# fircarpediem/LSS2_Multimodal_nu

Hardware: AMD Instinct MI355X
Metric: BEV frames/sec (6-cam 352x128 -> 200x200x64), full hot path: CamEncode lift + splat + BevEncode (higher is better)
Workload: dtype bf16; 1 GPU; BASELINE configs[1]: model_BEV_TXT LSS hot path, batch=4/GPU, 6 cams 352x128, D=41, 200x200x64 BEV -> BevEncode -> 200x200x4, trunk (EfficientNet) not included: features are the input; batch_per_gpu=4, global_batch=4, parallelism=dp1 (sample-sharded, no collective), precision=bf16

## Files before the change

include/lss_hip.h:

```cpp
#ifndef LSS_HIP_H_
#define LSS_HIP_H_

#include <stddef.h>
#include <stdint.h>

#ifdef __cplusplus
extern "C" {
#endif

#define LSS_ABI_VERSION 1

#define LSS_E_NULL (-1)
#define LSS_E_SHAPE (-2)
#define LSS_E_LAYOUT (-3)
#define LSS_E_ALIGN (-4)
#define LSS_E_WORKSPACE (-5)
#define LSS_E_RCCL_BASE (-100)

#define LSS_BEV_NCHW_F32 0
#define LSS_BEV_NHWC_F32 1
#define LSS_BEV_NHWC_BF16 2

#define LSS_DT_F32 0
#define LSS_DT_BF16 1
// ... 45 lines not shown
int lss_lift_splat_fwd(const float* feat, const int32_t* vox_list, const int32_t* entries,
                       int B, int N, int D, int fH, int fW, int C, int X, int Y, int Z,
                       void* bev, int layout, void* stream);

int lss_lift_splat_bwd(const void* grad_bev, int layout, const int32_t* voxel,
                       const float* depth, const float* feat, int B, int N, int D,
                       int fH, int fW, int C, int X, int Y, int Z, float* g_logits,
                       void* stream);

int lss_segmented_sum(const float* x, const int32_t* seg_start, int M, int C, float* y,
                      void* stream);

int lss_add_pos_fwd(const void* x, const float* pos, int B, int T, int C, int dt, void* q,
                    void* stream);

#define LSS_VALUE_NHWC 0
#define LSS_VALUE_HEAD_MAJOR 1
int lss_deform_attn_fwd(const void* value, int value_layout, const float* offsets_logits,
                        const float* token_bias, const float* ref_x, const float* ref_y, int B, int H,
                        int W, int n_heads, int n_points, int C, int dt, void* out, void* stream);

int lss_deform_attn_pts_fwd(const float* value, const float* offsets_logits, const float* ref_pts,
                            long long ref_bstride, int B, int H, int W, int n_heads, int n_points, int C,
                            float* out, void* stream);

int lss_deform_attn_bwd(const float* value, const float* offsets_logits, const float* ref_pts,
                        long long ref_bstride, const float* d_out, int B, int H, int W, int n_heads,
                        int n_points, int C, void* workspace, size_t workspace_bytes, float* d_value,
                        float* d_offsets_logits, void* stream);
size_t lss_deform_attn_bwd_workspace_bytes(int B, int H, int W);

int lss_layernorm_fwd(const void* x, int x_dt, const float* gamma, const float* beta,
                      long long rows, int C, float eps, void* y, int y_dt, void* stream);

size_t lss_conv2d_packed_weight_bytes(int Cout, int Cin, int KH, int KW, int dt);
int lss_conv2d_pack_weights(const float* w_oihw, int Cout, int Cin, int KH, int KW,
                            int dt, void* w_packed, void* stream);
int lss_conv2d_fwd(const void* x, const void* x2, const void* w_packed,
                   const float* scale, const float* shift, const void* residual,
                   void* y, float* stats, int B, int H, int W, int Cx, int C2, int up,
                   int Cout, int KH, int KW, int stride, int pad, int relu, int dt,
                   void* stream);

int lss_conv2d_ring_ok(int B, int H, int W, int Cx, int C2, int up, int Cout, int head_n);
size_t lss_conv2d_ring_packed_weight_bytes(int Cout, int Cin);
int lss_conv2d_pack_weights_ring(const float* w_oihw, int Cout, int Cin, void* w_packed, void* stream);
int lss_conv2d_pack_weights_ring_dgrad(const float* w_oihw, int Cout, int Cin, void* w_packed, void* stream);
int lss_conv2d_ring_timeouts(void);

int lss_conv2d_ks_ok(int B, int H, int W, int Cin, int Cout);
size_t lss_conv2d_ks_packed_weight_bytes(int Cout, int Cin);
int lss_conv2d_pack_weights_ks(const float* w_oihw, int Cout, int Cin, void* w_packed, void* stream);
int lss_conv2d_pack_weights_ks_dgrad(const float* w_oihw, int Cout, int Cin, void* w_packed, void* stream);

int lss_conv2d_pack_weights_dgrad(const float* w_oihw, int Cout, int Cin, int KH, int KW, int dt,
                                  void* w_packed, void* stream);
size_t lss_conv2d_wgrad_workspace_bytes(int B, int H, int W, int Cin, int Cout);
int lss_conv2d_wgrad(const void* x, const void* dy, int B, int H, int W, int Cin, int Cout,
                     void* workspace, size_t workspace_bytes, float* dw_oihw, void* stream);
int lss_conv2d_wgrad_timeouts(void);
int lss_conv2d_s2_dgrad_taps(int K, int pad);
int lss_conv2d_pack_weights_s2_dgrad(const float* w_oihw, int Cout, int Cin, int K, int pad, void* w_packed, void* stream);
size_t lss_conv2d_wgrad4x4_workspace_bytes(int B, int H, int W, int Cin, int Cout);
int lss_conv2d_wgrad4x4(const void* xs, const void* dy, int B, int H, int W, int Cin, int Cout,
                        void* workspace, size_t workspace_bytes, float* dw16, void* stream);

int lss_upsample_cat_nhwc(const void* x, const void* x2, int B, int H, int W, int Cx, int C2, int up,
                          void* out, void* stream);
int lss_upsample_bwd_nhwc(const void* g, int B, int H, int W, int Cx, int Ct, int c_off, int up,
                          void* dx, void* stream);

size_t lss_bn_train_workspace_bytes(long long M, int C);
int lss_bn_train_fwd(const void* z, const void* residual, long long M, int C, const float* gamma,
                     const float* beta, float* running_mean, float* running_var, float momentum,
                     float eps, int relu, void* workspace, void* y, float* save_mean,
                     float* save_invstd, void* stream);
int lss_bn_train_bwd(const void* dy, const void* y, const void* z, long long M, int C,
                     const float* gamma, const float* save_mean, const float* save_invstd, int relu,
                     void* workspace, void* dz, void* dres, float* dgamma, float* dbeta, void* stream);

int lss_bn_partial_sums(const void* z, const void* dy, const void* y, const float* mean, const float* invstd,
                        long long M, int C, int relu, int mode, void* workspace, float* sums, void* stream);
int lss_bn_train_fwd_from_sums(const void* z, const void* residual, long long M, int C, const float* sums,
                               long long M_total, const float* gamma, const float* beta, float* running_mean,
                               float* running_var, float momentum, float eps, int relu, void* workspace,
                               void* y, float* save_mean, float* save_invstd, void* stream);
int lss_bn_train_bwd_from_sums(const void* dy, const void* y, const void* z, long long M, int C,
                               const float* sums, long long M_total, const float* gamma,
                               const float* save_mean, const float* save_invstd, int relu, void* workspace,
                               void* dz, void* dres, float* dgamma, float* dbeta, void* stream);

int lss_conv_bn_act_train_fwd(const void* x1, const void* x2, const float* w_oihw, const float* gamma,
                              const float* beta, const void* residual, float* running_mean,
                              float* running_var, void* w_packed, void* z, void* y, float* save_mean,
                              float* save_invstd, void* bn_workspace, int B, int H, int W, int Cx, int C2,
                              int up, int Cout, float momentum, float eps, int relu, void* stream);
int lss_conv_bn_act_train_pack(const float* w_oihw, int B, int H, int W, int Cx, int C2, int up, int Cout, int dgrad,
                               void* w_packed, void* stream);
int lss_conv_bn_act_train_bwd(const void* dy, const void* y, const void* z, const void* x1, const void* x2,
                              const float* w_oihw, const float* gamma, const float* save_mean,
                              const float* save_invstd, void* bn_workspace, void* wgrad_workspace,
                              size_t wgrad_workspace_bytes, void* w_dgrad, void* dz, void* dres,
                              float* dgamma, float* dbeta, void* gcat, void* g1, void* xcat, float* dw,
                              int B, int H, int W, int Cx, int C2, int up, int Cout, int relu,
                              void* stream);

// ... 118 lines not shown
```

lss2_multimodal_nu_amd/_native.py:

```python
import ctypes
import os

import torch

_HERE = os.path.dirname(os.path.abspath(__file__))
LIB_PATH = os.environ.get("LSS_HIP_LIB") or os.path.join(_HERE, "csrc", "liblss_hip.so")

BEV_NCHW_F32, BEV_NHWC_F32, BEV_NHWC_BF16 = 0, 1, 2
DT_F32, DT_BF16 = 0, 1
ACT_NONE, ACT_RELU, ACT_GELU, OUT_F32, OUT_HEAD_MAJOR32, W_RING, W_KS = 0, 1, 2, 16, 32, 64, 128
VALUE_NHWC, VALUE_HEAD_MAJOR = 0, 1

_vp, _i, _sz = ctypes.c_void_p, ctypes.c_int, ctypes.c_size_t

SIGNATURES = {
    "lss_abi_version": (_i, []),
    "lss_error_string": (ctypes.c_char_p, [_i]),
    "lss_points_to_voxels": (_i, [_vp] * 7 + [_i] * 8 + [_vp, _vp, _vp, _vp]),
    "lss_geom_to_voxels": (_i, [_vp, _vp, _vp] + [_i] * 5 + [_vp, _vp, _vp]),
    "lss_bucket_points": (_i, [_vp, _vp, _i, _i, _i, _i, _vp, _vp, _vp, _vp, _vp]),
    "lss_depthnet_softmax_fwd": (_i, [_vp, _vp, _vp, _i, _i, _i, _i, _i, _vp, _vp, _i, _vp]),
    "lss_camencode_v2_fwd": (_i, [_vp, _i, _vp, _vp, _i, _vp, _vp, _vp] + [_i] * 7 + [_vp, _vp, _vp]),
    "lss_depth_fuse_softmax_fwd": (_i, [_vp] * 5 + [_i] * 6 + [_vp, _vp]),
    "lss_add_pos_fwd": (_i, [_vp, _vp, _i, _i, _i, _i, _vp, _vp]),
    "lss_deform_attn_fwd": (_i, [_vp, _i] + [_vp] * 4 + [_i] * 7 + [_vp, _vp]),
    "lss_deform_attn_pts_fwd": (_i, [_vp] * 3 + [ctypes.c_longlong] + [_i] * 6 + [_vp, _vp]),
    "lss_deform_attn_bwd": (_i, [_vp] * 3 + [ctypes.c_longlong, _vp] + [_i] * 6 + [_vp, _sz, _vp, _vp, _vp]),
    "lss_deform_attn_bwd_workspace_bytes": (_sz, [_i] * 3),
    "lss_layernorm_fwd": (_i, [_vp, _i, _vp, _vp, ctypes.c_longlong, _i, ctypes.c_float, _vp, _i, _vp]),
    "lss_depthnet_voxels_fwd": (_i, [_vp] * 10 + [_i] * 10 + [_vp] * 5),
    "lss_linear_res_ln_fwd": (_i, [_vp] * 4 + [ctypes.c_longlong, _i, _vp, _vp, _vp, ctypes.c_float, _vp, _vp]),
    "lss_ffn_fused_fwd": (_i, [_vp] * 5 + [ctypes.c_longlong, _i, _i, _vp, _vp, _vp, ctypes.c_float, _vp, _vp]),
    "lss_depthnet_voxels_hostcal_fwd": (_i, [_vp] * 7 + [_i] * 10 + [_vp] * 5),
    "lss_lift_splat_forward_hostcal": (_i, [_vp] * 7 + [_i] * 10 + [_vp] * 8 + [_i, _vp]),
    "lss_lift_splat_fwd": (_i, [_vp] * 3 + [_i] * 9 + [_vp, _i, _vp]),
    "lss_lift_splat_bwd": (_i, [_vp, _i, _vp, _vp, _vp] + [_i] * 9 + [_vp, _vp]),
    "lss_segmented_sum": (_i, [_vp, _vp, _i, _i, _vp, _vp]),
    "lss_conv2d_packed_weight_bytes": (_sz, [_i] * 5),
    "lss_conv2d_pack_weights": (_i, [_vp, _i, _i, _i, _i, _i, _vp, _vp]),
    "lss_conv2d_fwd": (_i, [_vp] * 8 + [_i] * 13 + [_vp]),
    "lss_conv2d_ring_ok": (_i, [_i] * 8),
    "lss_conv2d_ring_packed_weight_bytes": (_sz, [_i, _i]),
    "lss_conv2d_pack_weights_ring": (_i, [_vp, _i, _i, _vp, _vp]),
    "lss_conv2d_pack_weights_ring_dgrad": (_i, [_vp, _i, _i, _vp, _vp]),
    "lss_conv2d_ks_ok": (_i, [_i] * 5),
    "lss_conv2d_ks_packed_weight_bytes": (_sz, [_i, _i]),
    "lss_conv2d_pack_weights_ks": (_i, [_vp, _i, _i, _vp, _vp]),
    "lss_conv2d_pack_weights_ks_dgrad": (_i, [_vp, _i, _i, _vp, _vp]),
    "lss_gather_pack": (_i, [_vp, _i, _vp]),
    "lss_conv_bn_act_train_pack": (_i, [_vp] + [_i] * 8 + [_vp, _vp]),
    "lss_clip_adam_partials": (ctypes.c_longlong, [_vp, _i]),
    "lss_clip_adam_step": (_i, [_vp, _i, _vp, _vp, ctypes.c_longlong] + [ctypes.c_float] * 6 + [_vp]),
    "lss_conv2d_wgrad_timeouts": (_i, []),
    "lss_conv2d_ring_timeouts": (_i, []),
    "lss_conv2d_pack_weights_dgrad": (_i, [_vp, _i, _i, _i, _i, _i, _vp, _vp]),
    "lss_conv2d_wgrad_workspace_bytes": (_sz, [_i] * 5),
    "lss_conv2d_wgrad": (_i, [_vp, _vp, _i, _i, _i, _i, _i, _vp, _sz, _vp, _vp]),
    "lss_conv2d_wgrad4x4_workspace_bytes": (_sz, [_i] * 5),
    "lss_conv2d_s2_dgrad_taps": (_i, [_i, _i]),
    "lss_conv2d_pack_weights_s2_dgrad": (_i, [_vp, _i, _i, _i, _i, _vp, _vp]),
    "lss_conv2d_wgrad4x4": (_i, [_vp, _vp, _i, _i, _i, _i, _i, _vp, _sz, _vp, _vp]),
    "lss_upsample_cat_nhwc": (_i, [_vp, _vp, _i, _i, _i, _i, _i, _i, _vp, _vp]),
    "lss_upsample_bwd_nhwc": (_i, [_vp, _i, _i, _i, _i, _i, _i, _i, _vp, _vp]),
    "lss_bn_train_workspace_bytes": (_sz, [ctypes.c_longlong, _i]),
    "lss_bn_train_fwd": (_i, [_vp, _vp, ctypes.c_longlong, _i, _vp, _vp, _vp, _vp, ctypes.c_float, ctypes.c_float, _i,
                              _vp, _vp, _vp, _vp, _vp]),
    "lss_bn_train_bwd": (_i, [_vp, _vp, _vp, ctypes.c_longlong, _i, _vp, _vp, _vp, _i, _vp, _vp, _vp, _vp, _vp, _vp]),
    "lss_bn_partial_sums": (_i, [_vp] * 5 + [ctypes.c_longlong, _i, _i, _i, _vp, _vp, _vp]),
    "lss_bn_train_fwd_from_sums": (_i, [_vp, _vp, ctypes.c_longlong, _i, _vp, ctypes.c_longlong, _vp, _vp, _vp, _vp,
                                        ctypes.c_float, ctypes.c_float, _i, _vp, _vp, _vp, _vp, _vp]),
    "lss_bn_train_bwd_from_sums": (_i, [_vp, _vp, _vp, ctypes.c_longlong, _i, _vp, ctypes.c_longlong, _vp, _vp, _vp, _i,
                                        _vp, _vp, _vp, _vp, _vp, _vp]),
    "lss_conv_bn_act_train_fwd": (_i, [_vp] * 14 + [_i] * 7 + [ctypes.c_float, ctypes.c_float, _i, _vp]),
    "lss_conv_bn_act_train_bwd": (_i, [_vp] * 11 + [_sz] + [_vp] * 9 + [_i] * 8 + [_vp]),
    "lss_weighted_ce_fwd": (_i, [_vp, _vp, _vp, _i, _i, ctypes.c_longlong, _vp, _vp, _vp, _vp]),
    "lss_weighted_ce_bwd": (_i, [_vp, _vp, _vp, _i, _i, ctypes.c_longlong, _vp, _vp, _vp, _vp]),
    "lss_conv2d_s2d_packed_weight_bytes": (_sz, [_i] * 4),
    "lss_conv2d_pack_weights_s2d": (_i, [_vp, _i, _i, _i, _i, _vp, _vp]),
    "lss_conv2d_s2_fwd": (_i, [_vp] * 7 + [_i] * 8 + [_vp]),
    "lss_conv2d_head_fwd": (_i, [_vp] * 8 + [_i] * 9 + [_vp]),
    "lss_conv2d_s2_dual_fwd": (_i, [_vp] * 6 + [_i] * 9 + [_vp]),
    "lss_conv2d_sequence": (_i, [_vp, _i, _vp]),
    "lss_lift_splat_forward": (_i, [_vp] * 10 + [_i] * 10 + [_vp] * 8 + [_i, _i, _vp]),
    "lss_region_pipeline_ok": (_i, [_i] * 9),
    "lss_lift_splat_from_heads": (_i, [_vp] * 9 + [_i] * 9 + [_vp] * 6 + [_i, _vp]),
    "lss_lift_splat_direct_bytes": (_sz, [_i] * 9),
    "lss_lift_splat_forward_desc": (_i, [_vp, _vp]),
    "lss_head_ce_workspace_bytes": (_sz, [_i]),
    "lss_head_ce_fwd": (_i, [_vp] * 5 + [ctypes.c_longlong, _i, _i, _vp, _vp, _vp, _vp]),
    "lss_head_ce_bwd": (_i, [_vp] * 5 + [ctypes.c_longlong, _i, _i] + [_vp] * 7),
    "lss_head1x1_fwd": (_i, [_vp] * 3 + [ctypes.c_longlong, ctypes.c_longlong, _i, _i, _vp, _vp]),
    "lss_head1x1_bwd": (_i, [_vp] * 4 + [ctypes.c_longlong, ctypes.c_longlong, _i, _i] + [_vp] * 5),
    "lss_rccl_unique_id_bytes": (_sz, []),
    "lss_rccl_version": (_i, [_vp]),
    "lss_rccl_get_unique_id": (_i, [_vp]),
    "lss_rccl_comm_init": (_i, [_vp, _i, _i, _vp]),
    "lss_allreduce_bucket": (_i, [_vp, _vp, ctypes.c_longlong, _vp]),
    "lss_rccl_comm_destroy": (_i, [_vp]),
    "lss_nchw_f32_to_nhwc": (_i, [_vp, _vp, _i, _i, _i, _i, _i, _vp]),
    "lss_nhwc_to_nchw_f32": (_i, [_vp, _vp, _i, _i, _i, _i, _i, _vp]),
}
# ... 81 lines not shown
```

lss2_multimodal_nu_amd/csrc/conv_ks.hip:

```cpp
#include <stdlib.h>

#include "lss_common.h"

namespace {

constexpr int KS_ROWS = 7;
constexpr int KS_POSB = 64;
constexpr int KS_LDS_MAX = 160 * 1024;

__device__ __attribute__((aligned(128))) unsigned char lss_ks_zero_page[128];

__device__ __forceinline__ void ks_glds16(const void* gsrc, void* lds_wave_base) {
  __builtin_amdgcn_global_load_lds((const __attribute__((address_space(1))) void*)gsrc,
                                   (__attribute__((address_space(3))) void*)lds_wave_base, 16, 0, 0);
}

struct KsArgs {
  const unsigned short* x;
  const unsigned char* w;
  const float* scale;
  const float* shift;
  const unsigned short* residual;
  unsigned short* y;
  int B, H, W, Cin, Cout, relu, wt;
// ... 217 lines not shown
    const int cb = r / nks;
    const int m = l & 15, kq = l >> 4;
    const int co = cb * 32 + 8 * (m >> 2) + 4 * ct + (m & 3);
    const int ci = (S / 9) * 32 + kq * 8 + j;
    out[e] = lss_f2bf(dgrad ? w[((size_t)ci * Cout + co) * 9 + (8 - S % 9)] : w[((size_t)co * Cin + ci) * 9 + (S % 9)]);
  }
}

struct KsPlan {
  int ok, PB, npb, nposp, ncb, lds, grid, variant;
};

KsPlan ks_plan(int B, int H, int W, int Cin, int Cout) {
  KsPlan p = {};
  if (B <= 0 || H <= 0 || W < 4 || Cout <= 0 || Cout % 32 != 0) return p;
  if (Cin == 256) { p.variant = 0; p.PB = 80; }
  else if (Cin == 128) { p.variant = 1; p.PB = 160; }
  else if (Cin == 64) { p.variant = 2; p.PB = 320; }
  else return p;
  const long long HW = (long long)H * W;
  if (p.PB > 4 * W + 1) return p;
  p.npb = (int)((HW + p.PB - 1) / p.PB);
  p.ncb = Cout / 32;
  p.nposp = (KS_ROWS * (W + 2) + 31) / 32 * 32;
  const int patch = (Cin / 32) * p.nposp * KS_POSB;
  if (patch > 112 * 1024) return p;
  const int ntile = p.PB / 16;
  const int red = (p.variant == 2 ? 2 : 4) * ntile * 2 * 1024;
  p.lds = patch > red ? patch : red;
  if (p.lds > KS_LDS_MAX) return p;
  const long long grid = (long long)B * p.npb * p.ncb;
  if (grid < 64 || grid > 512) return p;
  if ((long long)B * HW * (Cin > Cout ? Cin : Cout) >= (1LL << 30)) return p;
  p.grid = (int)grid;
  p.ok = 1;
  return p;
}

template <int KSW, int NKW, int PXT>
int ks_launch(const KsPlan& p, const KsArgs& a, hipStream_t st) {
  static bool attr_set[64] = {};
  int dev = -1;
  if (hipGetDevice(&dev) != hipSuccess || dev < 0 || dev >= 64) dev = -1;
  if (dev < 0 || !attr_set[dev]) {
    hipError_t e = hipFuncSetAttribute(reinterpret_cast<const void*>(conv_ks_kernel<KSW, NKW, PXT>),
                                       hipFuncAttributeMaxDynamicSharedMemorySize, KS_LDS_MAX);
    if (e != hipSuccess) return (int)e;
    if (dev >= 0) attr_set[dev] = true;
  }
  hipLaunchKernelGGL((conv_ks_kernel<KSW, NKW, PXT>), dim3(p.grid), dim3(256), p.lds, st, a);
  return lss_launch_status();
}

}

extern "C" int lss_conv2d_ks_ok(int B, int H, int W, int Cin, int Cout) {
  if (const char* e = getenv("LSS_CONV_KS"))
    if (atoi(e) == 0) return 0;
  return ks_plan(B, H, W, Cin, Cout).ok;
}

extern "C" size_t lss_conv2d_ks_packed_weight_bytes(int Cout, int Cin) {
  if (Cout <= 0 || Cout % 32 != 0 || (Cin != 64 && Cin != 128 && Cin != 256)) return 0;
  return (size_t)Cout * Cin * 9 * 2;
}

extern "C" int lss_conv2d_pack_weights_ks(const float* w_oihw, int Cout, int Cin, void* w_packed, void* stream) {
  LSS_CHECK_PTR(w_oihw); LSS_CHECK_PTR(w_packed);
  if (lss_conv2d_ks_packed_weight_bytes(Cout, Cin) == 0) return LSS_E_SHAPE;
  const size_t n = (size_t)Cout * Cin * 9;
  const int grid = (int)((n + 255) / 256 > 4096 ? 4096 : (n + 255) / 256);
  hipLaunchKernelGGL(pack_weights_ks_kernel, dim3(grid), dim3(256), 0, lss_stream(stream), w_oihw, Cout, Cin,
                     reinterpret_cast<unsigned short*>(w_packed), 0);
  return lss_launch_status();
}

extern "C" int lss_conv2d_pack_weights_ks_dgrad(const float* w_oihw, int Cout, int Cin, void* w_packed, void* stream) {
  LSS_CHECK_PTR(w_oihw); LSS_CHECK_PTR(w_packed);
  if (lss_conv2d_ks_packed_weight_bytes(Cin, Cout) == 0) return LSS_E_SHAPE;
  const size_t n = (size_t)Cout * Cin * 9;
  const int grid = (int)((n + 255) / 256 > 4096 ? 4096 : (n + 255) / 256);
  hipLaunchKernelGGL(pack_weights_ks_kernel, dim3(grid), dim3(256), 0, lss_stream(stream), w_oihw, Cin, Cout,
                     reinterpret_cast<unsigned short*>(w_packed), 1);
  return lss_launch_status();
}

int lss_conv_ks_launch(const void* x, const void* w_ks, const float* scale, const float* shift, const void* residual,
                       void* y, int B, int H, int W, int Cin, int Cout, int relu, int wt, hipStream_t st) {
  const KsPlan p = ks_plan(B, H, W, Cin, Cout);
  if (!p.ok) return LSS_E_SHAPE;
  if (relu != 0 && relu != 1) return LSS_E_LAYOUT;
  if (((reinterpret_cast<uintptr_t>(x) | reinterpret_cast<uintptr_t>(y) | reinterpret_cast<uintptr_t>(w_ks) |
        reinterpret_cast<uintptr_t>(residual)) & 15) != 0)
    return LSS_E_ALIGN;
  KsArgs a;
  a.x = reinterpret_cast<const unsigned short*>(x);
  a.w = reinterpret_cast<const unsigned char*>(w_ks);
  a.scale = scale; a.shift = shift;
  a.residual = reinterpret_cast<const unsigned short*>(residual);
  a.y = reinterpret_cast<unsigned short*>(y);
  a.B = B; a.H = H; a.W = W; a.Cin = Cin; a.Cout = Cout; a.relu = relu; a.wt = wt;
  a.PB = p.PB; a.npb = p.npb; a.nposp = p.nposp; a.ncb = p.ncb;
  {
    const char* e = getenv("LSS_KS_STAMPS");
    a.stamps = e ? reinterpret_cast<unsigned long long*>(strtoull(e, nullptr, 16)) : nullptr;
  }
  if (p.variant == 0) return ks_launch<18, 4, 5>(p, a, st);
  if (p.variant == 1) return ks_launch<9, 4, 10>(p, a, st);
  return ks_launch<9, 2, 10>(p, a, st);
}
```

lss2_multimodal_nu_amd/csrc/conv_mfma.hip:

```cpp
#include <stdlib.h>

#include "lss_common.h"

int lss_linear_bf16_launch(const void* x, const void* w, const float* scale, const float* shift,
                           const void* residual, void* y, long long M, int N, int K, int act,
                           int out_f32, int group_hw, hipStream_t st);

int lss_conv_ring_launch(const void* x, const void* x2, const void* w_ring, const float* scale, const float* shift,
                         void* y, const float* head_w, const float* head_b, float* head_out, int head_n, int B, int H,
                         int W, int Cx, int C2, int up, int Cout, int relu, int wt, hipStream_t st);

int lss_conv_ks_launch(const void* x, const void* w_ks, const float* scale, const float* shift, const void* residual,
                       void* y, int B, int H, int W, int Cin, int Cout, int relu, int wt, hipStream_t st);

namespace {

struct ConvArgs {
  const void* x;
  const void* x2;
  const void* w;
  const float* scale;
  const float* shift;
  const void* residual;
  void* y;
// ... 1161 lines not shown
  a.y = nullptr; a.stats = nullptr;
  a.B = B; a.H = H; a.W = W; a.Cx = Cx; a.C2 = C2; a.up = up;
  a.Hin = H * up; a.Win = W * up; a.Cin = Cx + C2;
  a.Cout = Cout; a.KH = 3; a.KW = 3; a.stride = 1; a.pad = 1;
  a.Ho = a.Hin; a.Wo = a.Win;
  const long long M = (long long)B * a.Ho * a.Wo;
  if (M >= (1LL << 31)) return LSS_E_SHAPE;
  a.M = (int)M;
  a.relu = relu & 3;
  a.out_f32 = 0;
  a.wt = (getenv("LSS_CONV_WT") == nullptr || atoi(getenv("LSS_CONV_WT")) != 0) &&
         (unsigned long long)a.M * a.Cout * 2 < (1ULL << 31);
  a.y2 = nullptr; a.split = 0; a.relu_n = a.Cout;
  a.head_w = head_w; a.head_b = head_b; a.head_out = out; a.head_n = head_n;
  a.ry = a.Hin > 1 ? (float)(H - 1) / (float)(a.Hin - 1) : 0.f;
  a.rx = a.Win > 1 ? (float)(W - 1) / (float)(a.Win - 1) : 0.f;
  const bool fused = (up > 1) || (C2 > 0);
  const int tilesX = lss_cdiv(a.Wo, 16), tilesY = lss_cdiv(a.Ho, Cout == 64 ? 16 : 8);
  dim3 g(tilesX * tilesY * B, 1);
  hipStream_t st = lss_stream(stream);
  bool kc32 = fused && a.Cx % 32 == 0 && a.C2 % 32 == 0;
  if (const char* e = getenv("LSS_CONV_KC")) kc32 = kc32 && atoi(e) == 32;
  if (fused && kc32) {
    a.src_lds = conv_src_lds_ok(a);
    hipLaunchKernelGGL((conv_lds_kernel<2, 128, 1, 3, 3, 1, 32, 1, true>), g, dim3(256), 0, st, a, tilesX, tilesY);
  }
  else if (fused)
    hipLaunchKernelGGL((conv_lds_kernel<2, 128, 1, 3, 3, 1, 64, 1, true>), g, dim3(256), 0, st, a, tilesX, tilesY);
  else if (Cout == 64)
    hipLaunchKernelGGL((conv_lds_kernel<2, 64, 0, 3, 3, 1, 64, 1, true>), g, dim3(256), 0, st, a, tilesX, tilesY);
  else
    hipLaunchKernelGGL((conv_lds_kernel<2, 128, 0, 3, 3, 1, 64, 1, true>), g, dim3(256), 0, st, a, tilesX, tilesY);
  return lss_launch_status();
}

extern "C" int lss_conv2d_sequence(const lss_conv_launch_t* L, int n, void* stream) {
  LSS_CHECK_PTR(L);
  if (n < 0) return LSS_E_SHAPE;
  for (int i = 0; i < n; ++i) {
    const lss_conv_launch_t& c = L[i];
    int rc;
    if (c.kind == 0)
      rc = lss_conv2d_fwd(c.x, c.x2, c.w, c.scale, c.shift, c.residual, c.y, c.stats, c.B, c.H, c.W, c.Cx,
                          c.C2, c.up, c.Cout, c.KH, c.KW, c.stride, c.pad, c.relu, c.dt, stream);
    else if (c.kind == 1)
      rc = lss_conv2d_s2_fwd(c.x, c.w, c.scale, c.shift, c.residual, c.y, c.stats, c.B, c.H, c.W, c.Cx,
                             c.Cout, c.KH, c.pad, c.relu, stream);
    else if (c.kind == 2)
      rc = lss_conv2d_head_fwd(c.x, c.x2, c.w, c.scale, c.shift, c.head_w, c.head_b, c.head_out, c.B, c.H,
                               c.W, c.Cx, c.C2, c.up, c.Cout, c.head_n, c.relu, stream);
    else if (c.kind == 3)
      rc = lss_conv2d_s2_dual_fwd(c.x, c.w, c.scale, c.shift, c.y, c.y2, c.B, c.H, c.W, c.Cx, c.Cout, c.split, c.KH,
                                  c.pad, c.relu, stream);
    else
      rc = LSS_E_LAYOUT;
    if (rc != 0) return rc;
  }
  return 0;
}
```

lss2_multimodal_nu_amd/modules.py:

```python
import os

import torch
from torch import nn
from torch.nn import functional as F

from . import ops

_PRECISIONS = {"bf16": ops.DT_BF16, "fp32": ops.DT_F32}


def default_precision():
    p = os.environ.get("LSS_PRECISION", "bf16")
    if p not in _PRECISIONS:
        raise ValueError("LSS_PRECISION must be one of %s" % sorted(_PRECISIONS))
    return p


_warned_eval_autograd = set()


def _needs_autograd(module, *inputs):
    if not torch.is_grad_enabled():
        return False
    in_grad = any(t is not None and torch.is_tensor(t) and t.requires_grad for t in inputs)
# ... 628 lines not shown
    def forward(self, x):
        return self.get_eff_depth(x)

    def _load_from_state_dict(self, state_dict, prefix, local_metadata, strict, missing_keys, unexpected_keys,
                              error_msgs):
        if getattr(self, "trunk", None) is None:
            drop = [k for k in state_dict if k.startswith(prefix + "trunk.")]
            if drop:
                import warnings
                warnings.warn("%d '%strunk.*' checkpoint entries ignored: this Encoder was built without a trunk"
                              % (len(drop), prefix), stacklevel=3)
                for k in drop:
                    del state_dict[k]
        super()._load_from_state_dict(state_dict, prefix, local_metadata, strict, missing_keys, unexpected_keys,
                                      error_msgs)


class BasicBlock(nn.Module):

    def __init__(self, inplanes, planes, stride=1):
        super().__init__()
        self.conv1 = nn.Conv2d(inplanes, planes, 3, stride, 1, bias=False)
        self.bn1 = nn.BatchNorm2d(planes)
        self.relu = nn.ReLU(inplace=True)
        self.conv2 = nn.Conv2d(planes, planes, 3, 1, 1, bias=False)
        self.bn2 = nn.BatchNorm2d(planes)
        self.downsample = None
        if stride != 1 or inplanes != planes:
            self.downsample = nn.Sequential(nn.Conv2d(inplanes, planes, 1, stride, bias=False),
                                            nn.BatchNorm2d(planes))
        self._f1 = _FoldedConv(self.conv1, self.bn1)
        self._f2 = _FoldedConv(self.conv2, self.bn2)
        self._fd = _FoldedConv(self.downsample[0], self.downsample[1]) if self.downsample is not None else None

    def forward(self, x):
        idt = x if self.downsample is None else _train_bn_act(self.downsample[1], _train_conv(self.downsample[0], x), relu=False)
        out = _train_conv_bn_act(self.conv1, self.bn1, x, relu=True)
        return _train_conv_bn_act(self.conv2, self.bn2, out, relu=True, residual=idt)

    def _dual(self, dt):
        key = self._f1._key(dt) + self._fd._key(dt)
        if getattr(self, "_dual_key", None) != key:
            with torch.no_grad():
                w1, s1, b1 = self._f1.get(dt)
                _, sd, bd = self._fd.get(dt)
                wd = self.downsample[0].weight.detach().float()
                frame = wd.new_zeros(wd.shape[0], wd.shape[1], 3, 3)
                frame[:, :, 1, 1] = wd[:, :, 0, 0]
                self._dual_pack = (torch.cat([w1, ops.pack_conv_weight_s2d(frame.contiguous(), 1)], 1).contiguous(),
                                   torch.cat([s1, sd]).contiguous(), torch.cat([b1, bd]).contiguous())
            self._dual_key = key
        return self._dual_pack

    def _nhwc(self, x, dt):
        c1 = self.conv1
        if (self._fd is not None and dt == ops.DT_BF16 and c1.stride == (2, 2) and self._f1._s2d(dt)
                and self.downsample[0].stride == (2, 2) and c1.out_channels % 128 == 0
                and os.environ.get("LSS_NO_DUAL") is None):
            w, scale, shift = self._dual(dt)
            t, idt = ops.conv2d_s2_dual_nhwc(x, w, scale, shift, c1.out_channels, relu=True)
            return self._f2.run(t, dt, relu=True, residual=idt)
        idt = x if self._fd is None else self._fd.run(x, dt, relu=False)
        t = self._f1.run(x, dt, relu=True)
        return self._f2.run(t, dt, relu=True, residual=idt)


def _resnet18_layer(inplanes, planes, stride):
    return nn.Sequential(BasicBlock(inplanes, planes, stride), BasicBlock(planes, planes, 1))


class BevEncode(nn.Module):

    def __init__(self, inC, outC, precision=None):
        super().__init__()
        self.conv1 = nn.Conv2d(inC, 64, kernel_size=7, stride=2, padding=3, bias=False)
        self.bn1 = nn.BatchNorm2d(64)
        self.relu = nn.ReLU(inplace=True)
        self.layer1 = _resnet18_layer(64, 64, 1)
        self.layer2 = _resnet18_layer(64, 128, 2)
        self.layer3 = _resnet18_layer(128, 256, 2)
        for m in self.modules():
            if isinstance(m, nn.Conv2d):
                nn.init.kaiming_normal_(m.weight, mode="fan_out", nonlinearity="relu")
            elif isinstance(m, nn.BatchNorm2d):
                nn.init.constant_(m.weight, 1)
                nn.init.constant_(m.bias, 0)
        for m in self.modules():
            if isinstance(m, BasicBlock):
                nn.init.constant_(m.bn2.weight, 0)
        self.conv1.reset_parameters()
        self.up1 = Up(64 + 256, 256, scale_factor=4, precision=precision)
        self.up2 = nn.Sequential(
            nn.Upsample(scale_factor=2, mode="bilinear", align_corners=True),
            nn.Conv2d(256, 128, kernel_size=3, padding=1, bias=False),
            nn.BatchNorm2d(128),
            nn.ReLU(inplace=True),
            nn.Conv2d(128, outC, kernel_size=1, padding=0),
        )
        self.precision = precision
        self._plans = {}
        self._stem = _FoldedConv(self.conv1, self.bn1)
        self._up2a = _FoldedConv(self.up2[1], self.up2[2])
        self._up2b = _FoldedConv(self.up2[4], None)

    def features(self, x):
        if _native_training() and x.is_cuda:
            if x.dtype not in (torch.float32, torch.bfloat16):
                x = x.float()
            x = x.contiguous(memory_format=torch.channels_last)
        elif x.dtype != torch.float32:
            x = x.float()
        outer, _tls.counters = getattr(_tls, "counters", None), []
# ... 112 lines not shown
```

lss2_multimodal_nu_amd/ops.py:

```python
import ctypes
import os
import threading

import torch

from . import _native as N
from ._native import (ACT_GELU, ACT_NONE, ACT_RELU, BEV_NCHW_F32, BEV_NHWC_BF16, BEV_NHWC_F32, DT_BF16,
                      DT_F32, OUT_F32, OUT_HEAD_MAJOR32, VALUE_HEAD_MAJOR, VALUE_NHWC, W_KS, W_RING)


def _f32c(t, name, shape=None):
    if t.dtype != torch.float32 or not t.is_contiguous() or not t.is_cuda:
        raise ValueError("%s must be a contiguous fp32 GPU tensor (got %s %s contiguous=%s)"
                         % (name, t.dtype, t.device, t.is_contiguous()))
    if shape is not None and tuple(t.shape) != tuple(shape):
        raise ValueError("%s has shape %s, expected %s" % (name, tuple(t.shape), tuple(shape)))
    return t


class KernelTimer:

    def __init__(self, fine=False, last_conv=False):
        self.spans = {}
        self.fine = fine
# ... 1146 lines not shown
            "lss_conv2d_pack_weights_s2d")
    return out


def conv2d_s2_nhwc(x, w_s2d, K, pad, scale=None, shift=None, residual=None, relu=False, stats=None,
                   tag="conv2d_fwd"):
    B, H, W, Cx = x.shape
    taps, Cout, C4 = w_s2d.shape
    if x.dtype != torch.bfloat16 or not x.is_contiguous() or w_s2d.dtype != torch.bfloat16 \
            or C4 != (Cx if K == 1 else 4 * Cx):
        raise ValueError("conv2d_s2_nhwc operands must be contiguous bf16 with s2d-packed weights")
    Ho, Wo = (H + 2 * pad - K) // 2 + 1, (W + 2 * pad - K) // 2 + 1
    y = torch.empty(B, Ho, Wo, Cout, dtype=torch.bfloat16, device=x.device)
    for name, t in (("scale", scale), ("shift", shift)):
        if t is not None:
            _f32c(t, name, (Cout,))
    if residual is not None and (residual.dtype != torch.bfloat16 or tuple(residual.shape) != tuple(y.shape)
                                 or not residual.is_contiguous()):
        raise ValueError("residual must match the output")
    if stats is not None:
        _f32c(stats, "stats", (2 * Cout,))
    if _recorder is not None:
        _recorder.add(1, (x, w_s2d, scale, shift, residual, y, stats), x=x, w=w_s2d, scale=scale, shift=shift,
                      residual=residual, y=y, stats=stats, B=B, H=H, W=W, Cx=Cx, Cout=Cout, KH=K, KW=K, stride=2,
                      pad=pad, relu=1 if relu else 0, dt=DT_BF16)
    with _timed(tag):
        N.check(N.lib().lss_conv2d_s2_fwd(N.ptr(x), N.ptr(w_s2d), N.ptr(scale), N.ptr(shift), N.ptr(residual),
                                          N.ptr(y), N.ptr(stats), B, H, W, Cx, Cout, K, pad, 1 if relu else 0,
                                          N.stream()), "lss_conv2d_s2_fwd")
    return y


def conv2d_s2_dual_nhwc(x, w_s2d, scale, shift, split, relu=True, tag="conv2d_fwd"):
    B, H, W, Cx = x.shape
    taps, Cout, C4 = w_s2d.shape
    if x.dtype != torch.bfloat16 or not x.is_contiguous() or w_s2d.dtype != torch.bfloat16 or C4 != 4 * Cx:
        raise ValueError("conv2d_s2_dual_nhwc operands must be contiguous bf16 with s2d-packed weights")
    _f32c(scale, "scale", (Cout,))
    _f32c(shift, "shift", (Cout,))
    Ho, Wo = (H + 2 - 3) // 2 + 1, (W + 2 - 3) // 2 + 1
    y = torch.empty(B, Ho, Wo, split, dtype=torch.bfloat16, device=x.device)
    y2 = torch.empty(B, Ho, Wo, Cout - split, dtype=torch.bfloat16, device=x.device)
    if _recorder is not None:
        _recorder.add(3, (x, w_s2d, scale, shift, y, y2), x=x, w=w_s2d, scale=scale, shift=shift, y=y, y2=y2, B=B, H=H,
                      W=W, Cx=Cx, Cout=Cout, KH=3, KW=3, stride=2, pad=1, relu=1 if relu else 0, dt=DT_BF16,
                      split=split)
    with _timed(tag):
        N.check(N.lib().lss_conv2d_s2_dual_fwd(N.ptr(x), N.ptr(w_s2d), N.ptr(scale), N.ptr(shift), N.ptr(y), N.ptr(y2),
                                               B, H, W, Cx, Cout, split, 3, 1, 1 if relu else 0, N.stream()),
                "lss_conv2d_s2_dual_fwd")
    return y, y2


def conv3x3_head_nchw(x, w_packed, scale, shift, head_w, head_b, x2=None, up=1, relu=True, tag="conv2d_fwd"):
    B, H, W, Cx = x.shape
    ring = isinstance(w_packed, RingWeight)
    if ring:
        taps, Cout, Cin, w_packed = 9, w_packed.Cout, w_packed.Cin, w_packed.data
    else:
        taps, Cout, Cin = w_packed.shape
    C2 = x2.shape[3] if x2 is not None else 0
    if x.dtype != torch.bfloat16 or not x.is_contiguous() or taps != 9 or Cin != Cx + C2 or Cout not in (64, 128) \
            or (Cout == 64 and (up != 1 or C2 != 0)):
        raise ValueError("conv3x3_head_nchw: bf16 NHWC input, 3x3 weights with Cout == 128 (or 64 without "
                         "upsample / concat) required")
    n = head_w.shape[0]
    _f32c(head_w, "head_w", (n, Cout))
    _f32c(head_b, "head_b", (n,))
    _f32c(scale, "scale", (Cout,))
    _f32c(shift, "shift", (Cout,))
    out = torch.empty(B, n, H * up, W * up, dtype=torch.float32, device=x.device)
    if _recorder is not None:
        _recorder.add(2, (x, x2, w_packed, scale, shift, head_w, head_b, out), x=x, x2=x2, w=w_packed, scale=scale,
                      shift=shift, head_w=head_w, head_b=head_b, head_out=out, B=B, H=H, W=W, Cx=Cx, C2=C2, up=up,
                      Cout=Cout, KH=3, KW=3, stride=1, pad=1, relu=(1 if relu else 0) | (W_RING if ring else 0),
                      dt=DT_BF16, head_n=n)
    with _timed(tag):
        N.check(N.lib().lss_conv2d_head_fwd(N.ptr(x), N.ptr(x2), N.ptr(w_packed), N.ptr(scale), N.ptr(shift),
                                            N.ptr(head_w), N.ptr(head_b), N.ptr(out), B, H, W, Cx, C2, up, Cout, n,
                                            (1 if relu else 0) | (W_RING if ring else 0), N.stream()),
                "lss_conv2d_head_fwd")
    return out


def nchw_to_nhwc(x, dt):
    _f32c(x, "x")
    B, C, H, W = x.shape
    y = torch.empty(B, H, W, C, dtype=_TORCH_DT[dt], device=x.device)
    N.check(N.lib().lss_nchw_f32_to_nhwc(N.ptr(x), N.ptr(y), B, C, H, W, dt, N.stream()), "lss_nchw_f32_to_nhwc")
    return y


def nhwc_to_nchw(x, dt):
    if x.dtype != _TORCH_DT[dt] or not x.is_contiguous():
        raise ValueError("x must be contiguous %s" % _TORCH_DT[dt])
    B, H, W, C = x.shape
    y = torch.empty(B, C, H, W, dtype=torch.float32, device=x.device)
    N.check(N.lib().lss_nhwc_to_nchw_f32(N.ptr(x), N.ptr(y), B, C, H, W, dt, N.stream()), "lss_nhwc_to_nchw_f32")
    return y
```

Baseline: 11160 frames/s.

## Add KS-style fused stride-2 3x3 + 1x1 downsample dual conv kernel

Adds a new MFMA kernel that computes a stride-2 3x3 conv and its 1x1 downsample projection together. It stages an even/odd-column-split input patch in LDS via global_load_lds, splits K across waves, and reduces partials in LDS. It reuses the centre-tap fragments for the 1x1 product. The BasicBlock dual path uses it when the shape plan allows, replacing the previous s2d-based dual conv. The aim is to cut input traffic and raise MFMA efficiency for the ResNet layer2/3 transitions, at the cost of one block per CU (launch_bounds 256,1) and a narrow shape envelope.

```diff
diff --git a/include/lss_hip.h b/include/lss_hip.h
--- a/include/lss_hip.h
+++ b/include/lss_hip.h
@@ -121,6 +121,13 @@
 size_t lss_conv2d_ks_packed_weight_bytes(int Cout, int Cin);
 int lss_conv2d_pack_weights_ks(const float* w_oihw, int Cout, int Cin, void* w_packed, void* stream);
 int lss_conv2d_pack_weights_ks_dgrad(const float* w_oihw, int Cout, int Cin, void* w_packed, void* stream);
+
+int lss_conv2d_ks_s2_dual_ok(int B, int H, int W, int Cin, int Cout);
+size_t lss_conv2d_ks_s2_dual_packed_weight_bytes(int Cout, int Cin);
+int lss_conv2d_pack_weights_ks_s2_dual(const float* w1_oihw, const float* wd_oi, int Cout, int Cin, void* w_packed,
+                                       void* stream);
+int lss_conv2d_ks_s2_dual_fwd(const void* x, const void* w_packed, const float* scale, const float* shift, void* y,
+                              void* y2, int B, int H, int W, int Cin, int Cout, int relu, void* stream);
 
 int lss_conv2d_pack_weights_dgrad(const float* w_oihw, int Cout, int Cin, int KH, int KW, int dt,
                                   void* w_packed, void* stream);
diff --git a/lss2_multimodal_nu_amd/_native.py b/lss2_multimodal_nu_amd/_native.py
--- a/lss2_multimodal_nu_amd/_native.py
+++ b/lss2_multimodal_nu_amd/_native.py
@@ -47,6 +47,10 @@
     "lss_conv2d_ks_packed_weight_bytes": (_sz, [_i, _i]),
     "lss_conv2d_pack_weights_ks": (_i, [_vp, _i, _i, _vp, _vp]),
     "lss_conv2d_pack_weights_ks_dgrad": (_i, [_vp, _i, _i, _vp, _vp]),
+    "lss_conv2d_ks_s2_dual_ok": (_i, [_i] * 5),
+    "lss_conv2d_ks_s2_dual_packed_weight_bytes": (_sz, [_i, _i]),
+    "lss_conv2d_pack_weights_ks_s2_dual": (_i, [_vp, _vp, _i, _i, _vp, _vp]),
+    "lss_conv2d_ks_s2_dual_fwd": (_i, [_vp] * 6 + [_i] * 6 + [_vp]),
     "lss_gather_pack": (_i, [_vp, _i, _vp]),
     "lss_conv_bn_act_train_pack": (_i, [_vp] + [_i] * 8 + [_vp, _vp]),
     "lss_clip_adam_partials": (ctypes.c_longlong, [_vp, _i]),
diff --git a/lss2_multimodal_nu_amd/csrc/conv_ks.hip b/lss2_multimodal_nu_amd/csrc/conv_ks.hip
--- a/lss2_multimodal_nu_amd/csrc/conv_ks.hip
+++ b/lss2_multimodal_nu_amd/csrc/conv_ks.hip
@@ -293,6 +293,286 @@
   return lss_launch_status();
 }
 
+struct KsS2Args {
+  const unsigned short* x;
+  const unsigned char* w;
+  const float* scale;
+  const float* shift;
+  unsigned short* y;
+  unsigned short* y2;
+  int B, H, W, Cin, Cout, relu;
+  int Ho, Wo, pitch;
+  int PB, npb, nposp, ncb;
+  unsigned long long* stamps;
+};
+
+constexpr int KS2_PXT = 3;
+constexpr int KS2_CT = 4;
+
+template <int NKW>
+__global__ __launch_bounds__(256, 1) void conv_ks_s2_dual_kernel(const KsS2Args a) {
+  static_assert(NKW == 4 || NKW == 2, "one 32-channel chunk of nine taps per K part");
+  constexpr int NPW = 4 / NKW, PXT = KS2_PXT, CT = KS2_CT, NT = PXT * NPW, NCH = NKW;
+  extern __shared__ __attribute__((aligned(1024))) unsigned char smem[];
+  const int tid = threadIdx.x, lane = tid & 63;
+  const int wave = __builtin_amdgcn_readfirstlane(tid >> 6);
+  const int kp = wave % NKW, ph = wave / NKW;
+  const int n = lane & 15, kq = lane >> 4;
+  auto stamp = [&](int k) {
+    if (a.stamps != nullptr && tid == 0) a.stamps[(size_t)blockIdx.x * 8 + k] = __builtin_amdgcn_s_memrealtime();
+  };
+  stamp(0);
+  unsigned long long clk_main = 0;
+
+  int t;
+  {
+    const int nwg = gridDim.x, bid = blockIdx.x;
+    const int xcd = bid & 7, q8 = nwg >> 3, r8 = nwg & 7;
+    t = (xcd < r8 ? xcd * (q8 + 1) : r8 * (q8 + 1) + (xcd - r8) * q8) + (bid >> 3);
+  }
+  const int cb = t % a.ncb;
+  const int pbg = t / a.ncb;
+  const int b = pbg / a.npb, pb = pbg - b * a.npb;
+  const int HWo = a.Ho * a.Wo, WP = a.pitch;
+  const int p0 = pb * a.PB;
+  const int r0 = p0 / a.Wo;
+
+  {
+    const int ppc = a.nposp >> 4;
+    const int q64 = 64 / WP, r64 = 64 - q64 * WP;
+    const int h = wave & 1;
+    const int pos0 = 32 * (wave >> 1) + (lane >> 1);
+    int pr = pos0 / WP, pc = pos0 - pr * WP;
+    const unsigned char* zsrc = lss_ks_zero_page + (lane & 7) * 16;
+    const unsigned short* xb = a.x + (size_t)b * a.H * a.W * a.Cin + (2 * h + (lane & 1)) * 8;
+    for (int i = wave; i < ppc; i += 4) {
+      const int iy = 2 * r0 - 1 + pr, ix = pc < a.Wo ? 2 * pc : 2 * (pc - a.Wo) - 1;
+      const bool in = pr < KS_ROWS && iy >= 0 && iy < a.H && ix >= 0 && ix < a.W;
+      const unsigned short* src = xb + (in ? (iy * a.W + ix) * a.Cin : 0);
+#pragma unroll
+      for (int c = 0; c < NCH; ++c)
+        ks_glds16(in ? (const void*)(src + c * 32) : (const void*)zsrc,
+                  smem + ((size_t)(c * 2 + h) * a.nposp + 32 * (i >> 1)) * 32);
+      pr += q64; pc += r64;
+      if (pc >= WP) { pc -= WP; ++pr; }
+    }
+  }
+
+  constexpr int WPRE = 4;
+  bf16x8 wf[9][CT], wd[CT];
+  const unsigned char* wp = a.w + ((size_t)(cb * NKW + kp) * 10 * CT) * 1024 + lane * 16;
+  auto load_w = [&](int s) {
+#pragma unroll
+    for (int ct = 0; ct < CT; ++ct) wf[s][ct] = *reinterpret_cast<const bf16x8*>(wp + (s * CT + ct) * 1024);
+  };
+#pragma unroll
+  for (int s = 0; s < WPRE; ++s) load_w(s);
+#pragma unroll
+  for (int ct = 0; ct < CT; ++ct) wd[ct] = *reinterpret_cast<const bf16x8*>(wp + (9 * CT + ct) * 1024);
+
+  const int npx = min(a.PB, HWo - p0);
+  int ab[PXT];
+  {
+    const int x_first = p0 - r0 * a.Wo;
+    const int plast = npx - 1;
+    const int yl = (x_first + plast) / a.Wo, xl = x_first + plast - yl * a.Wo;
+    int pl = ph * PXT * 16 + n;
+    int y = (x_first + pl) / a.Wo, x = x_first + pl - y * a.Wo;
+#pragma unroll
+    for (int j = 0; j < PXT; ++j) {
+      const bool live = pl < npx;
+      ab[j] = (2 * (live ? y : yl) * WP + (live ? x : xl)) * 32 + (kq >> 1) * a.nposp * 32 + (kq & 1) * 16;
+      pl += 16; x += 16;
+      if (x >= a.Wo) { x -= a.Wo; ++y; }
+    }
+  }
+  stamp(1);
+  f32x4 acc[PXT][CT], acc2[PXT][CT];
+#pragma unroll
+  for (int j = 0; j < PXT; ++j)
+#pragma unroll
+    for (int ct = 0; ct < CT; ++ct) {
+      acc[j][ct] = (f32x4){0.f, 0.f, 0.f, 0.f};
+      acc2[j][ct] = (f32x4){0.f, 0.f, 0.f, 0.f};
+    }
+  asm volatile("s_waitcnt vmcnt(0)" ::: "memory");
+  __syncthreads();
+  stamp(2);
+
+  bf16x8 fb[2][PXT];
+  auto load_frags = [&](int buf, int s) {
+    const unsigned char* cbase = smem + (size_t)kp * a.nposp * KS_POSB;
+    const int ky = s / 3, kx = s % 3;
+    const int toff = (ky * WP + (kx == 1 ? 0 : kx == 0 ? a.Wo : a.Wo + 1)) * 32;
+#pragma unroll
+    for (int j = 0; j < PXT; ++j) fb[buf][j] = *reinterpret_cast<const bf16x8*>(cbase + ab[j] + toff);
+  };
+  if (a.stamps != nullptr) clk_main = __builtin_amdgcn_s_memtime();
+  load_frags(0, 0);
+#pragma unroll
+  for (int s = 0; s < 9; ++s) {
+    if (s + WPRE < 9) load_w(s + WPRE);
+    if (s + 1 < 9) load_frags((s + 1) & 1, s + 1);
+    __builtin_amdgcn_sched_barrier(0);
+#pragma unroll
+    for (int j = 0; j < PXT; ++j)
+#pragma unroll
+      for (int ct = 0; ct < CT; ++ct)
+        acc[j][ct] = __builtin_amdgcn_mfma_f32_16x16x32_bf16(wf[s][ct], fb[s & 1][j], acc[j][ct], 0, 0, 0);
+    if (s == 4) {
+#pragma unroll
+      for (int j = 0; j < PXT; ++j)
+#pragma unroll
+        for (int ct = 0; ct < CT; ++ct)
+          acc2[j][ct] = __builtin_amdgcn_mfma_f32_16x16x32_bf16(wd[ct], fb[0][j], acc2[j][ct], 0, 0, 0);
+    }
+    __builtin_amdgcn_sched_barrier(0);
+  }
+
+  if (a.stamps != nullptr) asm volatile("s_nop 0" ::"v"(acc[0][0]), "v"(acc[PXT - 1][CT - 1]));
+  stamp(3);
+  if (a.stamps != nullptr && tid == 0) a.stamps[(size_t)blockIdx.x * 8 + 7] = __builtin_amdgcn_s_memtime() - clk_main;
+  __syncthreads();
+  f32x4* part = reinterpret_cast<f32x4*>(smem);
+#pragma unroll
+  for (int j = 0; j < PXT; ++j) {
+    const int tile = ph * PXT + j;
+#pragma unroll
+    for (int ct = 0; ct < CT; ++ct) {
+      part[(((0 * NKW + kp) * NT + tile) * CT + ct) * 64 + lane] = acc[j][ct];
+      part[(((1 * NKW + kp) * NT + tile) * CT + ct) * 64 + lane] = acc2[j][ct];
+    }
+  }
+  float sc[2][2][8], sh[2][2][8];
+#pragma unroll
+  for (int o = 0; o < 2; ++o)
+#pragma unroll
+    for (int g = 0; g < 2; ++g) {
+      const int ch = o * a.Cout + cb * 64 + g * 32 + kq * 8;
+      f32x4 s0 = {1.f, 1.f, 1.f, 1.f}, s1 = s0, h0 = {0.f, 0.f, 0.f, 0.f}, h1 = h0;
+      if (a.scale) { s0 = *reinterpret_cast<const f32x4*>(a.scale + ch); s1 = *reinterpret_cast<const f32x4*>(a.scale + ch + 4); }
+      if (a.shift) { h0 = *reinterpret_cast<const f32x4*>(a.shift + ch); h1 = *reinterpret_cast<const f32x4*>(a.shift + ch + 4); }
+#pragma unroll
+      for (int i = 0; i < 4; ++i) { sc[o][g][i] = s0[i]; sc[o][g][4 + i] = s1[i]; sh[o][g][i] = h0[i]; sh[o][g][4 + i] = h1[i]; }
+    }
+  __syncthreads();
+  stamp(4);
+  constexpr int NOWN = (PXT + NKW - 1) / NKW;
+#pragma unroll
+  for (int k = 0; k < NOWN; ++k) {
+    const int j = kp + k * NKW;
+    if (j >= PXT) break;
+    const int tile = ph * PXT + j;
+    const int pl = tile * 16 + n;
+    const bool live = pl < npx;
+    const size_t opix = ((size_t)b * HWo + p0 + (live ? pl : 0)) * a.Cout + cb * 64 + kq * 8;
+#pragma unroll
+    for (int o = 0; o < 2; ++o)
+#pragma unroll
+      for (int g = 0; g < 2; ++g) {
+        float v[8];
+#pragma unroll
+        for (int tt = 0; tt < 2; ++tt) {
+          const int ct = 2 * g + tt;
+          f32x4 sum = part[(((o * NKW + 0) * NT + tile) * CT + ct) * 64 + lane];
+#pragma unroll
+          for (int q = 1; q < NKW; ++q) {
+            const f32x4 pv = part[(((o * NKW + q) * NT + tile) * CT + ct) * 64 + lane];
+#pragma unroll
+            for (int i = 0; i < 4; ++i) sum[i] += pv[i];
+          }
+#pragma unroll
+          for (int i = 0; i < 4; ++i) v[4 * tt + i] = sum[i];
+        }
+#pragma unroll
+        for (int i = 0; i < 8; ++i) {
+          v[i] = v[i] * sc[o][g][i] + sh[o][g][i];
+          if (o == 0 && a.relu) v[i] = fmaxf(v[i], 0.f);
+        }
+        if (live) {
+          typedef __attribute__((ext_vector_type(4))) unsigned int u32x4;
+          const u32x4 ov = {lss_pack_bf2(v[0], v[1]), lss_pack_bf2(v[2], v[3]), lss_pack_bf2(v[4], v[5]), lss_pack_bf2(v[6], v[7])};
+          *reinterpret_cast<u32x4*>((o == 0 ? a.y : a.y2) + opix + g * 32) = ov;
+        }
+      }
+  }
+  if (a.stamps != nullptr) {
+    stamp(5);
+    asm volatile("s_waitcnt vmcnt(0)" ::: "memory");
+    stamp(6);
+  }
+}
+
+__global__ void pack_weights_ks_s2_dual_kernel(const float* __restrict__ w1, const float* __restrict__ wd, int Cout,
+                                               int Cin, unsigned short* __restrict__ out) {
+  const size_t ntot = (size_t)Cout * Cin * 10;
+  const int nch = Cin >> 5;
+  for (size_t e = (size_t)blockIdx.x * 256 + threadIdx.x; e < ntot; e += (size_t)gridDim.x * 256) {
+    const int j = e & 7;
+    size_t r = e >> 3;
+    const int l = r & 63; r >>= 6;
+    const int ct = r & 3; r >>= 2;
+    const int s = r % 10; r /= 10;
+    const int kp = r % nch;
+    const int cb = r / nch;
+    const int m = l & 15, kq = l >> 4;
+    const int co = cb * 64 + 32 * (ct >> 1) + 8 * (m >> 2) + 4 * (ct & 1) + (m & 3);
+    const int ci = kp * 32 + kq * 8 + j;
+    out[e] = lss_f2bf(s < 9 ? w1[((size_t)co * Cin + ci) * 9 + s] : wd[(size_t)co * Cin + ci]);
+  }
+}
+
+struct KsS2Plan {
+  int ok, Ho, Wo, pitch, PB, npb, nposp, ncb, lds, grid, nkw;
+};
+
+KsS2Plan ks_s2_plan(int B, int H, int W, int Cin, int Cout) {
+  KsS2Plan p = {};
+  if (B <= 0 || H < 2 || W < 4 || Cout <= 0 || Cout % 64 != 0) return p;
+  if (Cin == 128) p.nkw = 4;
+  else if (Cin == 64) p.nkw = 2;
+  else return p;
+  p.Ho = (H - 1) / 2 + 1; p.Wo = (W - 1) / 2 + 1;
+  p.pitch = 2 * p.Wo + 1;
+  p.PB = 16 * KS2_PXT * (4 / p.nkw);
+  if (p.PB > 2 * p.Wo + 1) return p;
+  const long long HWo = (long long)p.Ho * p.Wo;
+  p.npb = (int)((HWo + p.PB - 1) / p.PB);
+  p.ncb = Cout / 64;
+  p.nposp = (KS_ROWS * p.pitch + 31) / 32 * 32;
+  const int patch = (Cin / 32) * p.nposp * KS_POSB;
+  if (patch > 112 * 1024) return p;
+  const int red = 2 * p.nkw * (p.PB / 16) * KS2_CT * 1024;
+  p.lds = patch > red ? patch : red;
+  if (p.lds > KS_LDS_MAX) return p;
+  const long long grid = (long long)B * p.npb * p.ncb;
+  if (grid < 64 || grid > 512) return p;
+  if ((long long)B * H * W * Cin >= (1LL << 30) || (long long)B * HWo * Cout >= (1LL << 30)) return p;
+  p.grid = (int)grid;
+  p.ok = 1;
+  return p;
+}
+
+template <int NKW>
+int ks_s2_launch(const KsS2Plan& p, const KsS2Args& a, hipStream_t st) {
+  static bool attr_set[64] = {};
+  int dev = -1;
+  if (hipGetDevice(&dev) != hipSuccess || dev < 0 || dev >= 64) dev = -1;
+  if (dev < 0 || !attr_set[dev]) {
+    hipError_t e = hipFuncSetAttribute(reinterpret_cast<const void*>(conv_ks_s2_dual_kernel<NKW>),
+                                       hipFuncAttributeMaxDynamicSharedMemorySize, KS_LDS_MAX);
+    if (e != hipSuccess) return (int)e;
+    if (dev >= 0) attr_set[dev] = true;
+  }
+  hipLaunchKernelGGL((conv_ks_s2_dual_kernel<NKW>), dim3(p.grid), dim3(256), p.lds, st, a);
+  return lss_launch_status();
+}
+
+unsigned long long* ks_stamps_from_env() {
+  const char* e = getenv("LSS_KS_STAMPS");
+  return e ? reinterpret_cast<unsigned long long*>(strtoull(e, nullptr, 16)) : nullptr;
+}
+
 }
 
 extern "C" int lss_conv2d_ks_ok(int B, int H, int W, int Cin, int Cout) {
@@ -342,11 +622,53 @@
   a.y = reinterpret_cast<unsigned short*>(y);
   a.B = B; a.H = H; a.W = W; a.Cin = Cin; a.Cout = Cout; a.relu = relu; a.wt = wt;
   a.PB = p.PB; a.npb = p.npb; a.nposp = p.nposp; a.ncb = p.ncb;
-  {
-    const char* e = getenv("LSS_KS_STAMPS");
-    a.stamps = e ? reinterpret_cast<unsigned long long*>(strtoull(e, nullptr, 16)) : nullptr;
-  }
+  a.stamps = ks_stamps_from_env();
   if (p.variant == 0) return ks_launch<18, 4, 5>(p, a, st);
   if (p.variant == 1) return ks_launch<9, 4, 10>(p, a, st);
   return ks_launch<9, 2, 10>(p, a, st);
 }
+
+extern "C" int lss_conv2d_ks_s2_dual_ok(int B, int H, int W, int Cin, int Cout) {
+  if (const char* e = getenv("LSS_CONV_KS"))
+    if (atoi(e) == 0) return 0;
+  return ks_s2_plan(B, H, W, Cin, Cout).ok;
+}
+
+extern "C" size_t lss_conv2d_ks_s2_dual_packed_weight_bytes(int Cout, int Cin) {
+  if (Cout <= 0 || Cout % 64 != 0 || (Cin != 64 && Cin != 128)) return 0;
+  return (size_t)Cout * Cin * 10 * 2;
+}
+
+extern "C" int lss_conv2d_pack_weights_ks_s2_dual(const float* w1_oihw, const float* wd_oi, int Cout, int Cin,
+                                                  void* w_packed, void* stream) {
+  LSS_CHECK_PTR(w1_oihw); LSS_CHECK_PTR(wd_oi); LSS_CHECK_PTR(w_packed);
+  if (lss_conv2d_ks_s2_dual_packed_weight_bytes(Cout, Cin) == 0) return LSS_E_SHAPE;
+  const size_t n = (size_t)Cout * Cin * 10;
+  const int grid = (int)((n + 255) / 256 > 4096 ? 4096 : (n + 255) / 256);
+  hipLaunchKernelGGL(pack_weights_ks_s2_dual_kernel, dim3(grid), dim3(256), 0, lss_stream(stream), w1_oihw, wd_oi, Cout,
+                     Cin, reinterpret_cast<unsigned short*>(w_packed));
+  return lss_launch_status();
+}
+
+extern "C" int lss_conv2d_ks_s2_dual_fwd(const void* x, const void* w_packed, const float* scale, const float* shift,
+                                         void* y, void* y2, int B, int H, int W, int Cin, int Cout, int relu,
+                                         void* stream) {
+  LSS_CHECK_PTR(x); LSS_CHECK_PTR(w_packed); LSS_CHECK_PTR(y); LSS_CHECK_PTR(y2);
+  const KsS2Plan p = ks_s2_plan(B, H, W, Cin, Cout);
+  if (!p.ok) return LSS_E_SHAPE;
+  if (relu != 0 && relu != 1) return LSS_E_LAYOUT;
+  if (((reinterpret_cast<uintptr_t>(x) | reinterpret_cast<uintptr_t>(y) | reinterpret_cast<uintptr_t>(y2) |
+        reinterpret_cast<uintptr_t>(w_packed) | reinterpret_cast<uintptr_t>(scale) | reinterpret_cast<uintptr_t>(shift)) & 15) != 0)
+    return LSS_E_ALIGN;
+  KsS2Args a;
+  a.x = reinterpret_cast<const unsigned short*>(x);
+  a.w = reinterpret_cast<const unsigned char*>(w_packed);
+  a.scale = scale; a.shift = shift;
+  a.y = reinterpret_cast<unsigned short*>(y);
+  a.y2 = reinterpret_cast<unsigned short*>(y2);
+  a.B = B; a.H = H; a.W = W; a.Cin = Cin; a.Cout = Cout; a.relu = relu;
+  a.Ho = p.Ho; a.Wo = p.Wo; a.pitch = p.pitch;
+  a.PB = p.PB; a.npb = p.npb; a.nposp = p.nposp; a.ncb = p.ncb;
+  a.stamps = ks_stamps_from_env();
+  return p.nkw == 4 ? ks_s2_launch<4>(p, a, lss_stream(stream)) : ks_s2_launch<2>(p, a, lss_stream(stream));
+}
diff --git a/lss2_multimodal_nu_amd/csrc/conv_mfma.hip b/lss2_multimodal_nu_amd/csrc/conv_mfma.hip
--- a/lss2_multimodal_nu_amd/csrc/conv_mfma.hip
+++ b/lss2_multimodal_nu_amd/csrc/conv_mfma.hip
@@ -1237,6 +1237,8 @@
     else if (c.kind == 3)
       rc = lss_conv2d_s2_dual_fwd(c.x, c.w, c.scale, c.shift, c.y, c.y2, c.B, c.H, c.W, c.Cx, c.Cout, c.split, c.KH,
                                   c.pad, c.relu, stream);
+    else if (c.kind == 4)
+      rc = lss_conv2d_ks_s2_dual_fwd(c.x, c.w, c.scale, c.shift, c.y, c.y2, c.B, c.H, c.W, c.Cx, c.Cout, c.relu, stream);
     else
       rc = LSS_E_LAYOUT;
     if (rc != 0) return rc;
diff --git a/lss2_multimodal_nu_amd/modules.py b/lss2_multimodal_nu_amd/modules.py
--- a/lss2_multimodal_nu_amd/modules.py
+++ b/lss2_multimodal_nu_amd/modules.py
@@ -704,12 +704,25 @@
             self._dual_key = key
         return self._dual_pack
 
+    def _dual_ks(self, dt):
+        if getattr(self, "_dual_ks_key", None) != self._dual_key:
+            with torch.no_grad():
+                self._dual_ks_pack = ops.pack_conv_weight_ks_s2_dual(
+                    self.conv1.weight.detach().float().contiguous(),
+                    self.downsample[0].weight.detach().float().contiguous())
+            self._dual_ks_key = self._dual_key
+        return self._dual_ks_pack
+
     def _nhwc(self, x, dt):
         c1 = self.conv1
         if (self._fd is not None and dt == ops.DT_BF16 and c1.stride == (2, 2) and self._f1._s2d(dt)
                 and self.downsample[0].stride == (2, 2) and c1.out_channels % 128 == 0
                 and os.environ.get("LSS_NO_DUAL") is None):
             w, scale, shift = self._dual(dt)
+            B, H, W, Cx = x.shape
+            if ops.conv_ks_s2_dual_ok(B, H, W, Cx, c1.out_channels):
+                t, idt = ops.conv2d_ks_s2_dual_nhwc(x, self._dual_ks(dt), scale, shift, relu=True)
+                return self._f2.run(t, dt, relu=True, residual=idt)
             t, idt = ops.conv2d_s2_dual_nhwc(x, w, scale, shift, c1.out_channels, relu=True)
             return self._f2.run(t, dt, relu=True, residual=idt)
         idt = x if self._fd is None else self._fd.run(x, dt, relu=False)
diff --git a/lss2_multimodal_nu_amd/ops.py b/lss2_multimodal_nu_amd/ops.py
--- a/lss2_multimodal_nu_amd/ops.py
+++ b/lss2_multimodal_nu_amd/ops.py
@@ -1222,6 +1222,46 @@
     return y, y2
 
 
+def conv_ks_s2_dual_ok(B, H, W, Cin, Cout):
+    return bool(N.lib().lss_conv2d_ks_s2_dual_ok(B, H, W, Cin, Cout))
+
+
+def pack_conv_weight_ks_s2_dual(w1_oihw, wd_oihw):
+    Cout, Cin, KH, KW = w1_oihw.shape
+    _f32c(w1_oihw, "conv weight")
+    _f32c(wd_oihw, "downsample weight", (Cout, Cin, 1, 1))
+    nbytes = N.lib().lss_conv2d_ks_s2_dual_packed_weight_bytes(Cout, Cin)
+    if (KH, KW) != (3, 3) or nbytes == 0:
+        raise ValueError("KS stride-2 weights: 3x3 + 1x1, Cout %% 64 == 0, Cin in (64, 128) (got %s)"
+                         % (tuple(w1_oihw.shape),))
+    out = torch.empty(nbytes // 2, dtype=torch.bfloat16, device=w1_oihw.device)
+    N.check(N.lib().lss_conv2d_pack_weights_ks_s2_dual(N.ptr(w1_oihw), N.ptr(wd_oihw), Cout, Cin, N.ptr(out),
+                                                       N.stream()), "lss_conv2d_pack_weights_ks_s2_dual")
+    return KsWeight(out, Cout, Cin)
+
+
+def conv2d_ks_s2_dual_nhwc(x, w_ks, scale=None, shift=None, relu=True, tag="conv2d_fwd"):
+    B, H, W, Cx = x.shape
+    if x.dtype != torch.bfloat16 or not x.is_contiguous() or not isinstance(w_ks, KsWeight) or w_ks.Cin != Cx \
+            or w_ks.data.numel() != w_ks.Cout * Cx * 10:
+        raise ValueError("conv2d_ks_s2_dual_nhwc operands must be contiguous bf16 with stride-2 KS-packed weights")
+    Cout = w_ks.Cout
+    for name, t in (("scale", scale), ("shift", shift)):
+        if t is not None:
+            _f32c(t, name, (2 * Cout,))
+    Ho, Wo = (H - 1) // 2 + 1, (W - 1) // 2 + 1
+    y = torch.empty(B, Ho, Wo, Cout, dtype=torch.bfloat16, device=x.device)
+    y2 = torch.empty(B, Ho, Wo, Cout, dtype=torch.bfloat16, device=x.device)
+    if _recorder is not None:
+        _recorder.add(4, (x, w_ks.data, scale, shift, y, y2), x=x, w=w_ks.data, scale=scale, shift=shift, y=y, y2=y2,
+                      B=B, H=H, W=W, Cx=Cx, Cout=Cout, KH=3, KW=3, stride=2, pad=1, relu=1 if relu else 0, dt=DT_BF16)
+    with _timed(tag):
+        N.check(N.lib().lss_conv2d_ks_s2_dual_fwd(N.ptr(x), N.ptr(w_ks.data), N.ptr(scale), N.ptr(shift), N.ptr(y),
+                                                  N.ptr(y2), B, H, W, Cx, Cout, 1 if relu else 0, N.stream()),
+                "lss_conv2d_ks_s2_dual_fwd")
+    return y, y2
+
+
 def conv3x3_head_nchw(x, w_packed, scale, shift, head_w, head_b, x2=None, up=1, relu=True, tag="conv2d_fwd"):
     B, H, W, Cx = x.shape
     ring = isinstance(w_packed, RingWeight)
```

Measured after the change: 11690 frames/s (median of 6 runs). 4.7% higher.
